# rsokolovskii/fl_scaling_sc_ldpc

Measured on AMD Instinct MI355X. Metric: MC codeword trials/sec, (4,8) SC-LDPC L=50 N=1000 eps=0.48 full BP, higher is better.
Workload: dtype u32

## Files before the change

### fl_scaling_sc_ldpc_amd/csrc/full_bp_small.hip

```cpp
#include "common.h"
#include "kernel_util.h"
#include <algorithm>
#include <cstdlib>
#include <type_traits>

namespace {

using namespace scldpc_dev;

enum { SC_NE = 0, SC_REM, SC_N0, SC_N1, SC_OVF, SC_Q, SC_N = 8 };
enum { LV_VALID = 2, LV_EXTRA0 = 3, LV_PUSH = 6, LV_DROP = 9, LV_REM = 12, LV_OVF = 15, LV_N = 18 };

struct SmArgs {
    int L, V, C, n, nk, cn_lim, nw, ncw;
    uint32_t magic_v, magic_c;
    int ntrials;
    int kswitch;
    int max_it;
    int rows_cap;
    int32_t *rows;
    int off_U, off_q0, off_q1, off_pos, off_scal, off_fb, total, qcap;
    const uint16_t *vn_adj16;
    const uint16_t *cn_adj16;
    const uint32_t *chan;
    int32_t *counters;
    uint32_t *erased_out;
    int ncaps;
    int caps[SCLDPC_MAX_CAPS];
};

template <int BLOCK, bool LEVEL, bool PERSIST, bool SOCK, bool TRAJ = false, bool CAPS = false, bool WIDE = false>
__global__ __launch_bounds__(BLOCK, WIDE ? 4 : PERSIST ? 8 : 7) __attribute__((amdgpu_num_sgpr(96))) void full_bp_small_kernel(const SmArgs a)
{
    static_assert(!WIDE || (BLOCK == 1024 && LEVEL && SOCK && !PERSIST && !CAPS), "the wide form: LEVEL [+ TRAJ], socket table");
    using QT = std::conditional_t<WIDE, uint32_t, uint16_t>;
    constexpr int kWaves = BLOCK / 64;
    extern __shared__ uint32_t lds[];
    uint32_t *cnt = lds;
    uint32_t *U = lds + a.off_U;
    QT *q[2] = {reinterpret_cast<QT *>(lds + a.off_q0), reinterpret_cast<QT *>(lds + a.off_q1)};
    int *pos_cnt = reinterpret_cast<int *>(lds + a.off_pos);
    int *pos_ss = pos_cnt + a.L;
    int *scal = reinterpret_cast<int *>(lds + a.off_scal);

    const int tid = threadIdx.x, lane = tid & 63, wave = tid >> 6;
    auto decode_trial = [&](const int trial) {
    STAMP_DECL
    const int n = a.n, nk = a.nk, cn_lim = a.cn_lim, nw = a.nw, V = a.V, C = a.C, L = a.L, qcap = a.qcap;
    const uint2 *vrow = reinterpret_cast<const uint2 *>(a.vn_adj16) + (size_t)trial * n;
    const uint4 *crow = reinterpret_cast<const uint4 *>(a.cn_adj16) + (size_t)trial * nk;
    const uint32_t *ch = a.chan + (size_t)trial * nw;

    for (int c = tid; c < a.ncw; c += BLOCK) cnt[c] = 0;
    int ne_local = 0;
    for (int w = tid; w < nw; w += BLOCK) {
        uint32_t x = ch[w];
        if (w == nw - 1 && (n & 31)) x &= (1u << (n & 31)) - 1u;
        U[w] = x;
        ne_local += __popc(x);
    }
    if (tid < LV_N) scal[tid] = 0;
    for (int i = tid; i < 2 * L; i += BLOCK) pos_cnt[i] = 0;
    __syncthreads();
    ne_local = wave_sum(ne_local);
    if (lane == 0 && ne_local) atomicAdd(&scal[SC_NE], ne_local);

    constexpr int NB = 8;
    for (int j0 = tid; j0 < n; j0 += NB * BLOCK) {
        uint2 r[NB];
        bool er[NB];
#pragma unroll
        for (int u = 0; u < NB; u++) {
            const int j = j0 + u * BLOCK;
            er[u] = false;
            if (j < n) { r[u] = vrow[j]; er[u] = (U[j >> 5] >> (j & 31)) & 1u; }
        }
#pragma unroll
        for (int u = 0; u < NB; u++) {
            const int j = j0 + u * BLOCK;
            if (er[u]) {
                const int base = (int)__umulhi((uint32_t)j, a.magic_v) * C;
                const int c0 = base + (int)(r[u].x & 0xFFFFu), c1 = base + C + (int)(r[u].x >> 16);
                const int c2 = base + 2 * C + (int)(r[u].y & 0xFFFFu), c3 = base + 3 * C + (int)(r[u].y >> 16);
                atomicAdd(&cnt[c0 >> 3], 1u << ((c0 & 7) * 4));
                atomicAdd(&cnt[c1 >> 3], 1u << ((c1 & 7) * 4));
                atomicAdd(&cnt[c2 >> 3], 1u << ((c2 & 7) * 4));
                atomicAdd(&cnt[c3 >> 3], 1u << ((c3 & 7) * 4));
            }
        }
    }
    __syncthreads();
    STAMP(0);
    const int nch = scal[SC_NE];

    int removed = 0, drops = 0;
    auto step = [&](int c, uint32_t (&out)[4]) {
        out[0] = out[1] = out[2] = out[3] = 0;
        const uint4 s4 = crow[c];
        uint32_t jk[8] = {s4.x & 0xFFFFu, s4.x >> 16, s4.y & 0xFFFFu, s4.y >> 16,
                          s4.z & 0xFFFFu, s4.z >> 16, s4.w & 0xFFFFu, s4.w >> 16};
        bool none[8];
#pragma unroll
        for (int k = 0; k < 8; k++) none[k] = jk[k] == 0xFFFFu;
        if constexpr (SOCK) {
            const int vbase = (int)__umulhi((uint32_t)c, a.magic_c) * V;
#pragma unroll
            for (int k = 0; k < 8; k++) jk[k] = (uint32_t)(vbase - (int)(jk[k] & 3u) * V) + (jk[k] >> 2);
        }
        uint32_t wd[8];
#pragma unroll
        for (int k = 0; k < 8; k++) wd[k] = U[none[k] ? 0u : jk[k] >> 5];
        int j = -1;
#pragma unroll
        for (int k = 0; k < 8; k++)
            if (!none[k] && ((wd[k] >> (jk[k] & 31u)) & 1u)) j = (int)jk[k];
        if (j < 0) return;
        const uint2 r = vrow[j];
        const uint32_t bit = 1u << (j & 31);
        if (!(atomicAnd(&U[j >> 5], ~bit) & bit)) return;
        removed++;
        const int base = (int)__umulhi((uint32_t)j, a.magic_v) * C;
        const int cc[4] = {base + (int)(r.x & 0xFFFFu), base + C + (int)(r.x >> 16),
                           base + 2 * C + (int)(r.y & 0xFFFFu), base + 3 * C + (int)(r.y >> 16)};
        uint32_t o[4];
#pragma unroll
        for (int i = 0; i < 4; i++) o[i] = atomicSub(&cnt[cc[i] >> 3], 1u << ((cc[i] & 7) * 4));
#pragma unroll
        for (int i = 0; i < 4; i++) {
            const uint32_t old = (o[i] >> ((cc[i] & 7) * 4)) & 15u;
            if (old == 2u && cc[i] < cn_lim) out[i] = (uint32_t)cc[i] + 1u;
            if constexpr (LEVEL) drops += (old == 1u && cc[i] < cn_lim);
        }
    };
    auto ones_of = [&](int w) {
        const uint32_t y = cnt[w] ^ 0x11111111u;
        uint32_t z = ~(((y & 0x77777777u) + 0x77777777u) | y) & 0x88888888u;
        if (w * 8 + 8 > cn_lim) {
            const int keep = cn_lim - w * 8;
            z = keep <= 0 ? 0u : (z & ((1u << (4 * keep)) - 1u));
        }
        return z;
    };
    auto append = [&](const uint32_t (&out)[4], int *push, QT *qn, bool &overflow) {
        const int mine = (out[0] != 0u) + (out[1] != 0u) + (out[2] != 0u) + (out[3] != 0u);
        const int incl = (int)wave_inclusive_scan((uint32_t)mine);
        const int tot = __builtin_amdgcn_readlane(incl, 63);
        if (tot) {
            int base = 0;
            if (lane == 0) base = atomicAdd(push, tot);
            int idx = __builtin_amdgcn_readfirstlane(base) + incl - mine;
#pragma unroll
            for (int i = 0; i < 4; i++)
                if (out[i]) { if (idx < qcap) qn[idx] = (QT)(out[i] - 1u); else overflow = true; idx++; }
        }
    };

    int rounds = 0, ne = 0, status = 0, be = 0, ee = 0, bee = 0;
    auto residual = [&]() {
    if (ne > 0) {
        for (int w = tid; w < nw; w += BLOCK) {
            uint32_t x = U[w];
            int p0 = (int)__umulhi((uint32_t)(w * 32), a.magic_v);
            int room = (p0 + 1) * V - w * 32;
            while (x) {
                const uint32_t lo = room >= 32 ? x : (x & ((1u << room) - 1u));
                if (lo) atomicAdd(&pos_cnt[p0], __popc(lo));
                x = room >= 32 ? 0u : (x >> room);
                p0++;
                room = V;
            }
        }
        __syncthreads();
        int q0 = 0;
        for (;;) {
            while (q0 < L && pos_cnt[q0] == 0) q0++;
            if (q0 >= L) break;
            for (int t = tid; t < V; t += BLOCK) {
                const int j = q0 * V + t;
                if (!((U[j >> 5] >> (j & 31)) & 1u)) continue;
                const uint2 r = vrow[j];
                const int base = q0 * C;
                const int cc[4] = {base + (int)(r.x & 0xFFFFu), base + C + (int)(r.x >> 16),
                                   base + 2 * C + (int)(r.y & 0xFFFFu), base + 3 * C + (int)(r.y >> 16)};
                bool pair = true;
#pragma unroll
                for (int i = 0; i < 4; i++) pair = pair && ((cnt[cc[i] >> 3] >> ((cc[i] & 7) * 4)) & 15u) == 2u;
                if (!pair) continue;
                int partner = -1;
                for (int i = 0; i < 4 && pair; i++) {
                    const uint4 s4 = crow[cc[i]];
                    const uint32_t jk[8] = {s4.x & 0xFFFFu, s4.x >> 16, s4.y & 0xFFFFu, s4.y >> 16,
                                            s4.z & 0xFFFFu, s4.z >> 16, s4.w & 0xFFFFu, s4.w >> 16};
                    int other = -1;
                    for (int k = 0; k < 8; k++) {
                        if (jk[k] == 0xFFFFu) continue;
                        const int j2 = SOCK ? (q0 + i - (int)(jk[k] & 3u)) * V + (int)(jk[k] >> 2) : (int)jk[k];
                        if (j2 != j && ((U[j2 >> 5] >> (j2 & 31)) & 1u)) other = j2;
                    }
                    if (other < 0 || (i > 0 && other != partner)) pair = false;
                    partner = other;
                }
                if (pair && (int)__umulhi((uint32_t)partner, a.magic_v) == q0) atomicAdd(&pos_ss[q0], 1);
            }
            __syncthreads();
            const int e = pos_cnt[q0] - pos_ss[q0];
            if (e > 0) { ee = e; bee = 1; break; }
            q0++;
        }
        for (int pos = 0; pos < L; pos++) be += pos_cnt[pos] > 0;
    }
    };
    auto put = [&](int32_t *o, int ne, int be, int ee, int bee, int rounds, int status) {
        o[SCLDPC_C_NUM_ERASURES] = ne;
        o[SCLDPC_C_NUM_BLOCKS_ERR] = be;
        o[SCLDPC_C_NUM_ERASURES_EXP] = ee;
        o[SCLDPC_C_NUM_BLOCKS_ERR_EXP] = bee;
        o[SCLDPC_C_NUM_ERASURES_P1] = 0;
        o[SCLDPC_C_ITERATIONS] = rounds;
        o[SCLDPC_C_STATUS] = status;
        o[SCLDPC_C_CHANNEL_ERASURES] = nch;
    };
    auto cap_counters = [&](int k) { return a.counters + ((size_t)k * a.ntrials + trial) * SCLDPC_NCOUNTERS; };

    int ci = 0;
    if constexpr (LEVEL) {
        uint8_t *fb = reinterpret_cast<uint8_t *>(lds + a.off_fb);
        int prec = n, iter = 0, ncur = 0, nfront = 0, first_word = 0;
        if constexpr (TRAJ) {
            int extra = 0;
            const int head = 3 * C, tail0 = L * C;
            for (int i = tid; i < 2 * head; i += BLOCK) {
                const int c = i < head ? i : tail0 + (i - head);
                if (c >= cn_lim || c >= nk) continue;
                const uint4 s4 = crow[c];
                const int deg = ((s4.x & 0xFFFFu) != 0xFFFFu) + ((s4.x >> 16) != 0xFFFFu) + ((s4.y & 0xFFFFu) != 0xFFFFu) +
                                ((s4.y >> 16) != 0xFFFFu) + ((s4.z & 0xFFFFu) != 0xFFFFu) + ((s4.z >> 16) != 0xFFFFu) +
                                ((s4.w & 0xFFFFu) != 0xFFFFu) + ((s4.w >> 16) != 0xFFFFu);
                extra += deg == 1 && ((cnt[c >> 3] >> ((c & 7) * 4)) & 15u) == 0u;
            }
            extra = wave_sum(extra);
            if (lane == 0 && extra) atomicAdd(&scal[LV_EXTRA0], extra);
        }
        bool scan = true;
        ne = nch;
        for (;;) {
            const int g = iter % 3, gn = (iter + 1) % 3;
            QT *qc = q[iter & 1], *qn = q[(iter + 1) & 1];
            if (tid == 0) { scal[LV_PUSH + gn] = 0; scal[LV_DROP + gn] = 0; scal[LV_REM + gn] = 0; scal[LV_OVF + gn] = 0; }
            int *push = &scal[LV_PUSH + g];
            bool overflow = false;
            removed = 0; drops = 0;
            auto run_queue = [&](int nq) {
                for (int k0 = wave * 64; k0 < nq; k0 += BLOCK) {
                    uint32_t out[4] = {0, 0, 0, 0};
                    if (k0 + lane < nq) step((int)qc[k0 + lane], out);
                    append(out, push, qn, overflow);
                }
            };
            if (scan) {
                int valid = 0;
                for (int w = tid; w < a.ncw; w += BLOCK) {
                    uint32_t y = ones_of(w) >> 3;
                    y = (y | (y >> 3)) & 0x03030303u;
                    y = (y | (y >> 6)) & 0x000F000Fu;
                    y = (y | (y >> 12)) & 0xFFu;
                    fb[w] = (uint8_t)y;
                    valid += __popc(y);
                }
                if (iter == 0) {
                    valid = wave_sum(valid);
                    if (lane == 0 && valid) atomicAdd(&scal[LV_VALID], valid);
                }
                if (tid == 0) scal[SC_Q] = 0;
                __syncthreads();
                if (iter == 0) nfront = scal[LV_VALID];
                for (;;) {
                    for (int w0 = wave * 64; w0 < a.ncw; w0 += BLOCK) {
                        const int w = w0 + lane;
                        uint32_t y = w < a.ncw ? (uint32_t)fb[w] : 0u;
                        const int mine = __popc(y);
                        const int incl = (int)wave_inclusive_scan((uint32_t)mine);
                        const int tot = __builtin_amdgcn_readlane(incl, 63);
                        if (tot == 0) continue;
                        int base = 0;
                        if (lane == 0) base = atomicAdd(&scal[SC_Q], tot);
                        int idx = __builtin_amdgcn_readfirstlane(base) + incl - mine;
                        uint32_t left = 0;
                        while (y) {
                            const int k = __ffs((int)y) - 1;
                            y &= y - 1;
                            if (idx < qcap) qc[idx] = (QT)(w * 8 + k); else left |= 1u << k;
                            idx++;
                        }
                        if (mine) fb[w] = (uint8_t)left;
                    }
                    __syncthreads();
                    const int found = scal[SC_Q];
                    __syncthreads();
                    if (tid == 0) scal[SC_Q] = 0;
                    run_queue(min(found, qcap));
                    if (found <= qcap) break;
                    __syncthreads();
                }
            } else {
                run_queue(ncur);
            }
            STAMP(4);
            {
                const uint32_t both = (uint32_t)wave_sum((int)((uint32_t)removed | ((uint32_t)drops << 15)));
                removed = (int)(both & 0x7FFFu); drops = (int)(both >> 15);
            }
            if (lane == 0) {
                if (removed) atomicAdd(&scal[LV_REM + g], removed);
                if (drops) atomicAdd(&scal[LV_DROP + g], drops);
            }
            if (overflow) scal[LV_OVF + g] = 1;
            STAMP(5);
            __syncthreads();
            STAMP(6);
            const int deg1 = nfront + ((TRAJ && iter == 0) ? scal[LV_EXTRA0] : 0);
            ne -= scal[LV_REM + g];
            const int recovered = prec - ne;
            if constexpr (TRAJ) {
                if (wave == 0 && a.rows && rounds < a.rows_cap) {
                    int fw = first_word, first = n;
                    while (fw < nw) {
                        const uint32_t w = (fw + lane < nw) ? U[fw + lane] : 0u;
                        const unsigned long long m = __ballot(w != 0u);
                        if (m) {
                            const int l0 = __ffsll((long long)m) - 1;
                            const uint32_t w0 = (uint32_t)__shfl((int)w, l0, 64);
                            fw += l0;
                            first = fw * 32 + (__ffs((int)w0) - 1);
                            break;
                        }
                        fw += 64;
                    }
                    first_word = fw;
                    if (lane == 0) {
                        int32_t *r = a.rows + ((size_t)trial * a.rows_cap + rounds) * 3;
                        r[0] = deg1; r[1] = recovered; r[2] = (int)__umulhi((uint32_t)first, a.magic_v);
                    }
                }
                __syncthreads();
            }
            rounds++;
            if (deg1 < recovered && iter > 0) { status = -1; break; }
            if (ne == 0 || ne == prec) break;
            prec = ne;
            nfront = scal[LV_PUSH + g] - (scal[LV_DROP + g] - nfront);
            scan = scal[LV_OVF + g] != 0;
            ncur = scan ? 0 : scal[LV_PUSH + g];
            iter++;
            if (!CAPS && a.max_it > 0 && iter >= a.max_it) break;
            if constexpr (CAPS) {
                if (iter >= a.caps[ci]) {
                    be = ee = bee = 0;
                    residual();
                    if (tid == 0) put(cap_counters(ci), ne, be, ee, bee, rounds, 0);
                    __syncthreads();
                    for (int i = tid; i < 2 * L; i += BLOCK) pos_cnt[i] = 0;
                    if (++ci == a.ncaps) break;
                }
            }
            STAMP(7);
        }
        __syncthreads();
        STAMP(1);
    } else {
        const int kSwitch = a.kswitch;
        const int wcap = (qcap / kWaves) & ~1, half_cap = wcap / 2;
        int ncur = 0;
        bool scan = true;
        for (;;) {
            QT *qc = q[rounds & 1], *qn = q[(rounds + 1) & 1];
            if (scan) {
                for (int w0 = wave * 64; w0 < a.ncw; w0 += BLOCK) {
                    const int w = w0 + lane;
                    uint32_t z = w < a.ncw ? ones_of(w) : 0u;
                    const int mine = __popc(z);
                    const int incl = (int)wave_inclusive_scan((uint32_t)mine);
                    const int tot = __builtin_amdgcn_readlane(incl, 63);
                    if (tot == 0) continue;
                    int base = 0;
                    if (lane == 0) base = atomicAdd(&scal[SC_Q], tot);
                    base = __builtin_amdgcn_readfirstlane(base);
                    int idx = base + incl - mine;
                    while (z) {
                        const int k = (__ffs((int)z) - 1) >> 2;
                        z &= z - 1;
                        if (idx < qcap) qc[idx] = (QT)(w * 8 + k);
                        idx++;
                    }
                }
                __syncthreads();
                ncur = scal[SC_Q];
                if (ncur > qcap) { ncur = qcap; if (tid == 0) scal[SC_OVF] = 1; }
                __syncthreads();
            }
            if (tid == 0) { scal[SC_Q] = 0; scal[SC_N0 + ((rounds + 1) & 1)] = 0; }
            int *push = &scal[SC_N0 + (rounds & 1)];
            bool overflow = false;
            if (ncur > kSwitch || half_cap < 64) {
                for (int k0 = wave * 64; k0 < ncur; k0 += BLOCK) {
                    uint32_t out[4] = {0, 0, 0, 0};
                    if (k0 + lane < ncur) step((int)qc[k0 + lane], out);
                    append(out, push, qn, overflow);
                }
            } else {
                QT *mine = qn + wave * wcap;
                int cntw = (ncur - wave + kWaves - 1) / kWaves, cur = 0;
                if (cntw < 0) cntw = 0;
                if (lane < cntw) mine[lane] = qc[wave + lane * kWaves];
                while (cntw > 0) {
                    QT *src = mine + cur * half_cap, *dst = mine + (cur ^ 1) * half_cap;
                    int ncnt = 0;
                    for (int b0 = 0; b0 < cntw; b0 += 64) {
                        uint32_t out[4] = {0, 0, 0, 0};
                        if (b0 + lane < cntw) step((int)src[b0 + lane], out);
                        {
                            const int mine_n = (out[0] != 0u) + (out[1] != 0u) + (out[2] != 0u) + (out[3] != 0u);
                            const int incl = (int)wave_inclusive_scan((uint32_t)mine_n);
                            int idx = ncnt + incl - mine_n;
    #pragma unroll
                            for (int i = 0; i < 4; i++)
                                if (out[i]) { if (idx < half_cap) dst[idx] = (QT)(out[i] - 1u); else overflow = true; idx++; }
                            ncnt += __builtin_amdgcn_readlane(incl, 63);
                        }
                    }
                    cntw = min(ncnt, half_cap);
                    cur ^= 1;
                }
            }
            if (overflow) scal[SC_OVF] = 1;
            __syncthreads();
            rounds++;
            const int pushed = *push;
            scan = scal[SC_OVF] != 0;
            __syncthreads();
            if (tid == 0) scal[SC_OVF] = 0;
            ncur = scan ? 0 : min(pushed, qcap);
            if (!scan && ncur == 0) break;
        }
        STAMP(1);
        removed = wave_sum(removed);
        if (lane == 0 && removed) atomicAdd(&scal[SC_REM], removed);
        __syncthreads();
        ne = nch - scal[SC_REM];
    }

    if (!CAPS || ci < a.ncaps) {
        be = ee = bee = 0;
        residual();
    }
    STAMP(2);
    STAMP_FLUSH();
    if (a.erased_out)
        for (int w = tid; w < nw; w += BLOCK) a.erased_out[(size_t)trial * nw + w] = U[w];
    if (tid == 0) {
        if constexpr (CAPS) {
            for (int k = ci; k < a.ncaps; k++) put(cap_counters(k), ne, be, ee, bee, rounds, status);
        } else {
            put(a.counters + (size_t)trial * SCLDPC_NCOUNTERS, ne, be, ee, bee, rounds, status);
        }
    }
    };
    if constexpr (PERSIST) {
        for (int trial = blockIdx.x; trial < a.ntrials; trial += gridDim.x) {
            decode_trial(trial);
            __syncthreads();
        }
    } else {
        decode_trial((int)blockIdx.x);
    }
}

int make_args(const scldpc_code_params *p, int32_t is_term, SmArgs *a, int per_cu, bool level = false, bool wide = false)
{
    const int n = scldpc::n_of(p), nk = scldpc::nk_of(p);
    a->L = p->L; a->V = p->vns_pos; a->C = p->cns_pos; a->n = n; a->nk = nk;
    a->cn_lim = is_term ? nk : p->L * p->cns_pos;
    a->nw = (n + 31) / 32; a->ncw = (nk + 7) / 8;
    int off = 0;
    auto take = [&](int words) { int o = off; off += (words + 3) & ~3; return o; };
    take(a->ncw);
    a->off_U = take(a->nw);
    a->off_pos = take(2 * p->L);
    a->off_scal = take(LV_N);
    a->off_fb = level ? take((a->ncw + 3) / 4) : 0;
    const int budget = scldpc::kMaxLdsBytes / per_cu / 4 - 128;
    int qwords = ((budget - off) / 2) & ~3;
    if (qwords > 2048 && !wide) qwords = 2048;
    if (qwords < 128) return -1;
    a->qcap = wide ? qwords : 2 * qwords;
    a->off_q0 = take(qwords);
    a->off_q1 = take(qwords);
    a->total = off;
    return 0;
}

constexpr int kBlockSmall = 256;
constexpr int kPerCu = 7;
constexpr int kSwitchWidth = 128;
constexpr int kBlockWide = 1024;
constexpr int kWideMinQueue = 1024;
static_assert(kSwitchWidth <= 64 * (kBlockSmall / 64), "a wave takes at most one frontier entry per lane into its private queue");

}

namespace {
bool small_shape(const scldpc_code_params *p)
{
    if (scldpc::check_params(p)) return false;
    SmArgs a{};
    uint32_t m;
    return p->dv == 4 && p->dc == 8 && p->cns_pos <= 65536 && scldpc::nk_of(p) <= 65536 &&
           make_args(p, 1, &a, 1) == 0 && scldpc::magic_of(p->vns_pos, scldpc::n_of(p) + 32, &m) &&
           scldpc::magic_of(p->cns_pos, scldpc::nk_of(p), &m);
}
}

namespace {
const char *wide_limit(const scldpc_code_params *p)
{
    if (scldpc::check_params(p)) return "invalid code parameters";
    if (p->dv != 4 || p->dc != 8) return "takes dv = 4, dc = 8 only";
    if ((int64_t)p->vns_pos * p->dv > 65535) return "sockets: vns_pos * dv must fit 16 bits (at most 65535)";
    if (p->cns_pos > 65536) return "sockets: at most 65536 CNs per position (16-bit position-local CN ids)";
    const int64_t n64 = (int64_t)p->L * p->vns_pos, nk64 = (int64_t)(p->L + p->dv - 1) * p->cns_pos;
    if (n64 / 8 + nk64 / 2 > scldpc::kMaxLdsBytes) return "LDS: the CN counts and VN bits of a trial exceed 160 KiB";
    SmArgs a{};
    uint32_t m;
    if (!scldpc::magic_of(p->vns_pos, scldpc::n_of(p) + 32, &m) || !scldpc::magic_of(p->cns_pos, scldpc::nk_of(p), &m))
        return "no exact multiply-high division for this vns_pos / cns_pos";
    if (make_args(p, 1, &a, 1, true, true) != 0) return "LDS: the CN counts and VN bits of a trial leave no room for the queues";
    if (a.qcap < kWideMinQueue) return "queue: the LDS left by the state holds fewer than 1024 entries per queue";
    if (a.nk / 16 + 64 * (a.nk / a.qcap + 1) > 32767) return "queue: a wave's releases per iteration could exceed 15 bits";
    return nullptr;
}
}

extern "C" int scldpc_full_bp_wide_supported(const scldpc_code_params *p)
{
    return wide_limit(p) == nullptr;
}

extern "C" int scldpc_full_bp_cn16_supported(const scldpc_code_params *p)
{
    return small_shape(p) && scldpc::n_of(p) < 65535;
}

extern "C" int scldpc_full_bp_sock16_supported(const scldpc_code_params *p)
{
    return small_shape(p) && (int64_t)p->vns_pos * p->dv <= 65535;
}

namespace {

int launch_small(const char *who, bool level, bool sock, const scldpc_code_params *p, int32_t ntrials, const uint16_t *d_vn_adj16,
                 const uint16_t *d_cn_adj16, const uint32_t *d_chan_bits, int32_t max_it, int32_t is_term,
                 int32_t *d_counters, uint32_t *d_erased_bits, void *stream, int32_t *d_rows = nullptr, int32_t rows_cap = 0)
{
    if (d_rows && (rows_cap <= 0 || !level))
        return scldpc::set_error(SCLDPC_ERR_BAD_ARG, "%s: d_rows given but rows_cap <= 0", who);
    if (int rc = scldpc::check_params(p)) return rc;
    if (!(sock ? scldpc_full_bp_sock16_supported(p) : scldpc_full_bp_cn16_supported(p)))
        return scldpc::set_error(SCLDPC_ERR_TOO_LARGE, "%s: takes dv = 4, dc = 8, at most 65536 CNs per trial%s", who,
                                 sock ? " and 16-bit sockets" : " and fewer than 65535 VNs (use the _sock16 form beyond)");
    if (ntrials < 0 || (ntrials > 0 && (!d_counters || !d_vn_adj16 || !d_cn_adj16 || !d_chan_bits)))
        return scldpc::set_error(SCLDPC_ERR_BAD_ARG, "%s: null buffer or negative ntrials", who);
    if (ntrials == 0) return SCLDPC_OK;
    SmArgs a{};
    int per_cu = kPerCu;
    while (per_cu > 1 && make_args(p, is_term, &a, per_cu, level) != 0) per_cu--;
    if (make_args(p, is_term, &a, per_cu, level) != 0)
        return scldpc::set_error(SCLDPC_ERR_TOO_LARGE, "%s: the CN counts and VN bits do not fit the LDS", who);
    scldpc::magic_of(p->vns_pos, a.n + 32, &a.magic_v);
    scldpc::magic_of(p->cns_pos, a.nk, &a.magic_c);
    a.vn_adj16 = d_vn_adj16; a.cn_adj16 = d_cn_adj16; a.chan = d_chan_bits;
    a.counters = d_counters; a.erased_out = d_erased_bits;
    a.kswitch = kSwitchWidth;
    if (const char *v = getenv("SCLDPC_DEBUG_DECODER_KSWITCH")) a.kswitch = std::min(atoi(v), 64 * (kBlockSmall / 64));
    a.ntrials = ntrials;
    a.rows = d_rows; a.rows_cap = d_rows ? rows_cap : 0;
    a.max_it = max_it;
    const int grid = scldpc::debug_grid("DECODER", ntrials);
    void (*kern)(const SmArgs) = sock ? (level ? full_bp_small_kernel<kBlockSmall, true, false, true> : full_bp_small_kernel<kBlockSmall, false, false, true>)
        : grid < ntrials ? (level ? full_bp_small_kernel<kBlockSmall, true, true, false> : full_bp_small_kernel<kBlockSmall, false, true, false>)
                         : (level ? full_bp_small_kernel<kBlockSmall, true, false, false> : full_bp_small_kernel<kBlockSmall, false, false, false>);
    if (sock && grid < ntrials) return scldpc::set_error(SCLDPC_ERR_BAD_ARG, "%s: no persistent form with the socket table", who);
    if (d_rows) kern = sock ? full_bp_small_kernel<kBlockSmall, true, false, true, true> : full_bp_small_kernel<kBlockSmall, true, false, false, true>;
    size_t lds_bytes = 4u * (size_t)a.total;
    lds_bytes = std::min(lds_bytes + scldpc::debug_lds_pad("DECODER"), (size_t)scldpc::kMaxLdsBytes);
    if (int rc_ = scldpc::allow_max_lds(reinterpret_cast<const void *>(kern))) return rc_;
    hipLaunchKernelGGL(kern, dim3(grid), dim3(kBlockSmall), lds_bytes, static_cast<hipStream_t>(stream), a);
    SCLDPC_HIP_CHECK(hipGetLastError());
    return SCLDPC_OK;
}

int launch_caps(const char *who, bool sock, const scldpc_code_params *p, int32_t ntrials, const uint16_t *d_vn_adj16,
                const uint16_t *d_cn_adj16, const uint32_t *d_chan_bits, int32_t ncaps, const int32_t *caps, int32_t is_term,
                int32_t *d_counters, void *stream)
{
    if (ncaps < 1 || ncaps > SCLDPC_MAX_CAPS || !caps)
        return scldpc::set_error(SCLDPC_ERR_BAD_ARG, "%s: takes 1 .. %d caps (ncaps = %d%s)", who, SCLDPC_MAX_CAPS, ncaps,
                                 caps ? "" : ", caps NULL");
    for (int k = 0; k < ncaps; k++)
        if (caps[k] < 1 || (k > 0 && caps[k] <= caps[k - 1]))
            return scldpc::set_error(SCLDPC_ERR_BAD_ARG, "%s: caps must be strictly increasing and >= 1 (caps[%d] = %d)", who, k,
                                     caps[k]);
    if (ntrials < 0 || (ntrials > 0 && (!d_counters || !d_vn_adj16 || !d_cn_adj16 || !d_chan_bits)))
        return scldpc::set_error(SCLDPC_ERR_BAD_ARG, "%s: null buffer or negative ntrials", who);
    if (int rc = scldpc::check_params(p)) return rc;
    if (!(sock ? scldpc_full_bp_sock16_supported(p) : scldpc_full_bp_cn16_supported(p)))
        return scldpc::set_error(SCLDPC_ERR_TOO_LARGE, "%s: takes dv = 4, dc = 8, at most 65536 CNs per trial%s", who,
                                 sock ? " and 16-bit sockets" : " and fewer than 65535 VNs (use the _sock16 form beyond)");
    if (ntrials == 0) return SCLDPC_OK;
    SmArgs a{};
    int per_cu = kPerCu;
    while (per_cu > 1 && make_args(p, is_term, &a, per_cu, true) != 0) per_cu--;
    if (make_args(p, is_term, &a, per_cu, true) != 0)
        return scldpc::set_error(SCLDPC_ERR_TOO_LARGE, "%s: the CN counts and VN bits do not fit the LDS", who);
    scldpc::magic_of(p->vns_pos, a.n + 32, &a.magic_v);
    scldpc::magic_of(p->cns_pos, a.nk, &a.magic_c);
    a.vn_adj16 = d_vn_adj16; a.cn_adj16 = d_cn_adj16; a.chan = d_chan_bits;
    a.counters = d_counters;
    a.kswitch = kSwitchWidth;
    a.ntrials = ntrials;
    a.ncaps = ncaps;
    for (int k = 0; k < ncaps; k++) a.caps[k] = caps[k];
    void (*kern)(const SmArgs) = sock ? full_bp_small_kernel<kBlockSmall, true, false, true, false, true>
                                      : full_bp_small_kernel<kBlockSmall, true, false, false, false, true>;
    const size_t lds_bytes = 4u * (size_t)a.total;
    if (int rc_ = scldpc::allow_max_lds(reinterpret_cast<const void *>(kern))) return rc_;
    hipLaunchKernelGGL(kern, dim3(ntrials), dim3(kBlockSmall), lds_bytes, static_cast<hipStream_t>(stream), a);
    SCLDPC_HIP_CHECK(hipGetLastError());
    return SCLDPC_OK;
}

int launch_wide(const char *who, const scldpc_code_params *p, int32_t ntrials, const uint16_t *d_vn_adj16,
                const uint16_t *d_cn_sock16, const uint32_t *d_chan_bits, int32_t max_it, int32_t is_term,
                int32_t *d_counters, uint32_t *d_erased_bits, void *stream, int32_t *d_rows, int32_t rows_cap)
{
    if (d_rows && rows_cap <= 0) return scldpc::set_error(SCLDPC_ERR_BAD_ARG, "%s: d_rows given but rows_cap <= 0", who);
    if (int rc = scldpc::check_params(p)) return rc;
    if (const char *why = wide_limit(p)) return scldpc::set_error(SCLDPC_ERR_TOO_LARGE, "%s: %s", who, why);
    if (ntrials < 0 || (ntrials > 0 && (!d_counters || !d_vn_adj16 || !d_cn_sock16 || !d_chan_bits)))
        return scldpc::set_error(SCLDPC_ERR_BAD_ARG, "%s: null buffer or negative ntrials", who);
    if (ntrials == 0) return SCLDPC_OK;
    SmArgs a{};
    if (make_args(p, is_term, &a, 1, true, true) != 0 || 4u * (size_t)a.total > (size_t)scldpc::kMaxLdsBytes)
        return scldpc::set_error(SCLDPC_ERR_TOO_LARGE, "%s: LDS: the CN counts and VN bits do not fit", who);
    scldpc::magic_of(p->vns_pos, a.n + 32, &a.magic_v);
    scldpc::magic_of(p->cns_pos, a.nk, &a.magic_c);
    a.vn_adj16 = d_vn_adj16; a.cn_adj16 = d_cn_sock16; a.chan = d_chan_bits;
    a.counters = d_counters; a.erased_out = d_erased_bits;
    a.kswitch = kSwitchWidth;
    a.ntrials = ntrials;
    a.rows = d_rows; a.rows_cap = d_rows ? rows_cap : 0;
    a.max_it = max_it;
    void (*kern)(const SmArgs) = d_rows ? full_bp_small_kernel<kBlockWide, true, false, true, true, false, true>
                                        : full_bp_small_kernel<kBlockWide, true, false, true, false, false, true>;
    const size_t lds_bytes = 4u * (size_t)a.total;
    if (int rc_ = scldpc::allow_max_lds(reinterpret_cast<const void *>(kern))) return rc_;
    hipLaunchKernelGGL(kern, dim3(ntrials), dim3(kBlockWide), lds_bytes, static_cast<hipStream_t>(stream), a);
    SCLDPC_HIP_CHECK(hipGetLastError());
    return SCLDPC_OK;
}

}

extern "C" int scldpc_full_bp_device_wide(const scldpc_code_params *p, int32_t ntrials, const uint16_t *d_vn_adj16,
                                          const uint16_t *d_cn_sock16, const uint32_t *d_chan_bits, int32_t max_it,
                                          int32_t is_term, int32_t *d_counters, uint32_t *d_erased_bits, void *stream)
{
    return launch_wide("scldpc_full_bp_device_wide", p, ntrials, d_vn_adj16, d_cn_sock16, d_chan_bits, max_it, is_term,
                       d_counters, d_erased_bits, stream, nullptr, 0);
}

extern "C" int scldpc_full_bp_traj_device_wide(const scldpc_code_params *p, int32_t ntrials, const uint16_t *d_vn_adj16,
                                               const uint16_t *d_cn_sock16, const uint32_t *d_chan_bits, int32_t max_it,
                                               int32_t is_term, int32_t *d_counters, int32_t *d_rows, int32_t rows_cap,
                                               uint32_t *d_erased_bits, void *stream)
{
    if (!d_rows) return scldpc::set_error(SCLDPC_ERR_BAD_ARG, "scldpc_full_bp_traj_device_wide: null d_rows");
    return launch_wide("scldpc_full_bp_traj_device_wide", p, ntrials, d_vn_adj16, d_cn_sock16, d_chan_bits, max_it, is_term,
                       d_counters, d_erased_bits, stream, d_rows, rows_cap);
}

extern "C" int scldpc_full_bp_fixpoint_device_cn16(const scldpc_code_params *p, int32_t ntrials,
                                                   const uint16_t *d_vn_adj16, const uint16_t *d_cn_adj16,
                                                   const uint32_t *d_chan_bits, int32_t is_term, int32_t *d_counters,
                                                   uint32_t *d_erased_bits, void *stream)
{
    return launch_small("scldpc_full_bp_fixpoint_device_cn16", false, false, p, ntrials, d_vn_adj16, d_cn_adj16, d_chan_bits, 0,
                        is_term, d_counters, d_erased_bits, stream);
}

extern "C" int scldpc_full_bp_device_cn16(const scldpc_code_params *p, int32_t ntrials, const uint16_t *d_vn_adj16,
                                          const uint16_t *d_cn_adj16, const uint32_t *d_chan_bits, int32_t max_it,
                                          int32_t is_term, int32_t *d_counters, uint32_t *d_erased_bits, void *stream)
{
    return launch_small("scldpc_full_bp_device_cn16", true, false, p, ntrials, d_vn_adj16, d_cn_adj16, d_chan_bits, max_it,
                        is_term, d_counters, d_erased_bits, stream);
}

extern "C" int scldpc_full_bp_fixpoint_device_sock16(const scldpc_code_params *p, int32_t ntrials,
                                                     const uint16_t *d_vn_adj16, const uint16_t *d_cn_sock16,
                                                     const uint32_t *d_chan_bits, int32_t is_term, int32_t *d_counters,
                                                     uint32_t *d_erased_bits, void *stream)
{
    return launch_small("scldpc_full_bp_fixpoint_device_sock16", false, true, p, ntrials, d_vn_adj16, d_cn_sock16, d_chan_bits,
                        0, is_term, d_counters, d_erased_bits, stream);
}

extern "C" int scldpc_full_bp_device_sock16(const scldpc_code_params *p, int32_t ntrials, const uint16_t *d_vn_adj16,
                                            const uint16_t *d_cn_sock16, const uint32_t *d_chan_bits, int32_t max_it,
                                            int32_t is_term, int32_t *d_counters, uint32_t *d_erased_bits, void *stream)
{
    return launch_small("scldpc_full_bp_device_sock16", true, true, p, ntrials, d_vn_adj16, d_cn_sock16, d_chan_bits, max_it,
                        is_term, d_counters, d_erased_bits, stream);
}

extern "C" int scldpc_full_bp_traj_device_cn16(const scldpc_code_params *p, int32_t ntrials, const uint16_t *d_vn_adj16,
                                               const uint16_t *d_cn_adj16, const uint32_t *d_chan_bits, int32_t max_it,
                                               int32_t is_term, int32_t *d_counters, int32_t *d_rows, int32_t rows_cap,
                                               uint32_t *d_erased_bits, void *stream)
{
    if (!d_rows) return scldpc::set_error(SCLDPC_ERR_BAD_ARG, "scldpc_full_bp_traj_device_cn16: null d_rows");
    return launch_small("scldpc_full_bp_traj_device_cn16", true, false, p, ntrials, d_vn_adj16, d_cn_adj16, d_chan_bits, max_it,
                        is_term, d_counters, d_erased_bits, stream, d_rows, rows_cap);
}

extern "C" int scldpc_full_bp_traj_device_sock16(const scldpc_code_params *p, int32_t ntrials, const uint16_t *d_vn_adj16,
                                                 const uint16_t *d_cn_sock16, const uint32_t *d_chan_bits, int32_t max_it,
                                                 int32_t is_term, int32_t *d_counters, int32_t *d_rows, int32_t rows_cap,
                                                 uint32_t *d_erased_bits, void *stream)
{
    if (!d_rows) return scldpc::set_error(SCLDPC_ERR_BAD_ARG, "scldpc_full_bp_traj_device_sock16: null d_rows");
    return launch_small("scldpc_full_bp_traj_device_sock16", true, true, p, ntrials, d_vn_adj16, d_cn_sock16, d_chan_bits, max_it,
                        is_term, d_counters, d_erased_bits, stream, d_rows, rows_cap);
}

extern "C" int scldpc_full_bp_caps_device_cn16(const scldpc_code_params *p, int32_t ntrials, const uint16_t *d_vn_adj16,
                                               const uint16_t *d_cn_adj16, const uint32_t *d_chan_bits, int32_t ncaps,
                                               const int32_t *caps, int32_t is_term, int32_t *d_counters, void *stream)
{
    return launch_caps("scldpc_full_bp_caps_device_cn16", false, p, ntrials, d_vn_adj16, d_cn_adj16, d_chan_bits, ncaps, caps,
                       is_term, d_counters, stream);
}

extern "C" int scldpc_full_bp_caps_device_sock16(const scldpc_code_params *p, int32_t ntrials, const uint16_t *d_vn_adj16,
                                                 const uint16_t *d_cn_sock16, const uint32_t *d_chan_bits, int32_t ncaps,
                                                 const int32_t *caps, int32_t is_term, int32_t *d_counters, void *stream)
{
    return launch_caps("scldpc_full_bp_caps_device_sock16", true, p, ntrials, d_vn_adj16, d_cn_sock16, d_chan_bits, ncaps, caps,
                       is_term, d_counters, stream);
}
```

Measured before the change: 1.218 million.

## Build CN erasure counts per check row and seed peeling queue with degree-one VNs

In the non-level, non-socket fixpoint form, the initial CN erasure counters are now built by each thread reading its check-node row, gathering the erased bits of its neighbours, and packing eight 4-bit counts per word with DPP lane merges. This replaces the per-erased-VN atomicAdd scatter. The same pass finds degree-one checks and writes their single erased VN id straight into the first queue, so the first peeling round skips the counter scan and starts from a VN list. The cost is reading every CN row even when few VNs are erased, plus a new template variant. An environment variable can switch back to the old build.

Result: no change. 1.221 million, median of 6 (+0.3%).

```diff
diff --git a/fl_scaling_sc_ldpc_amd/csrc/full_bp_small.hip b/fl_scaling_sc_ldpc_amd/csrc/full_bp_small.hip
--- a/fl_scaling_sc_ldpc_amd/csrc/full_bp_small.hip
+++ b/fl_scaling_sc_ldpc_amd/csrc/full_bp_small.hip
@@ -2,13 +2,14 @@
 #include "kernel_util.h"
 #include <algorithm>
 #include <cstdlib>
+#include <cstring>
 #include <type_traits>
 
 namespace {
 
 using namespace scldpc_dev;
 
-enum { SC_NE = 0, SC_REM, SC_N0, SC_N1, SC_OVF, SC_Q, SC_N = 8 };
+enum { SC_NE = 0, SC_REM, SC_N0, SC_N1, SC_OVF, SC_Q, SC_B, SC_N = 8 };
 enum { LV_VALID = 2, LV_EXTRA0 = 3, LV_PUSH = 6, LV_DROP = 9, LV_REM = 12, LV_OVF = 15, LV_N = 18 };
 
 struct SmArgs {
@@ -29,10 +30,11 @@
     int caps[SCLDPC_MAX_CAPS];
 };
 
-template <int BLOCK, bool LEVEL, bool PERSIST, bool SOCK, bool TRAJ = false, bool CAPS = false, bool WIDE = false>
+template <int BLOCK, bool LEVEL, bool PERSIST, bool SOCK, bool TRAJ = false, bool CAPS = false, bool WIDE = false, bool CNB = false>
 __global__ __launch_bounds__(BLOCK, WIDE ? 4 : PERSIST ? 8 : 7) __attribute__((amdgpu_num_sgpr(96))) void full_bp_small_kernel(const SmArgs a)
 {
     static_assert(!WIDE || (BLOCK == 1024 && LEVEL && SOCK && !PERSIST && !CAPS), "the wide form: LEVEL [+ TRAJ], socket table");
+    static_assert(!CNB || (!LEVEL && !SOCK && !WIDE && BLOCK % 64 == 0), "the CN-row build: fixpoint form, 16-bit VN ids as queue entries");
     using QT = std::conditional_t<WIDE, uint32_t, uint16_t>;
     constexpr int kWaves = BLOCK / 64;
     extern __shared__ uint32_t lds[];
@@ -51,7 +53,8 @@
     const uint4 *crow = reinterpret_cast<const uint4 *>(a.cn_adj16) + (size_t)trial * nk;
     const uint32_t *ch = a.chan + (size_t)trial * nw;
 
-    for (int c = tid; c < a.ncw; c += BLOCK) cnt[c] = 0;
+    if constexpr (!CNB)
+        for (int c = tid; c < a.ncw; c += BLOCK) cnt[c] = 0;
     int ne_local = 0;
     for (int w = tid; w < nw; w += BLOCK) {
         uint32_t x = ch[w];
@@ -65,6 +68,65 @@
     ne_local = wave_sum(ne_local);
     if (lane == 0 && ne_local) atomicAdd(&scal[SC_NE], ne_local);
 
+    if constexpr (CNB) {
+    constexpr int NB = 4;
+    QT *q0 = q[0];
+    const int nk8 = a.ncw * 8;
+    for (int b = 0; b < nk8; b += NB * BLOCK) {
+        uint4 r[NB];
+#pragma unroll
+        for (int u = 0; u < NB; u++) {
+            const int c = b + u * BLOCK + tid;
+            r[u] = make_uint4(~0u, ~0u, ~0u, ~0u);
+            if (c < nk) r[u] = crow[c];
+        }
+        auto tally = [&](auto full, const uint4 &s4, uint32_t &count, uint32_t &j1) {
+            const uint32_t jk[8] = {s4.x & 0xFFFFu, s4.x >> 16, s4.y & 0xFFFFu, s4.y >> 16,
+                                    s4.z & 0xFFFFu, s4.z >> 16, s4.w & 0xFFFFu, s4.w >> 16};
+            uint32_t wd[8];
+#pragma unroll
+            for (int k = 0; k < 8; k++) wd[k] = U[(decltype(full)::value || jk[k] != 0xFFFFu) ? jk[k] >> 5 : 0u];
+            count = 0; j1 = 0;
+#pragma unroll
+            for (int k = 0; k < 8; k++) {
+                const bool set = (decltype(full)::value || jk[k] != 0xFFFFu) && ((wd[k] >> (jk[k] & 31u)) & 1u);
+                count += set;
+                j1 = set ? jk[k] : j1;
+            }
+        };
+        bool one[NB];
+        uint32_t j1[NB];
+#pragma unroll
+        for (int u = 0; u < NB; u++) {
+            const int c = b + u * BLOCK + tid;
+            const int cw = b + u * BLOCK + __builtin_amdgcn_readfirstlane(wave) * 64;
+            uint32_t count;
+            if (cw >= 3 * C && cw + 64 <= L * C) tally(std::true_type{}, r[u], count, j1[u]);
+            else tally(std::false_type{}, r[u], count, j1[u]);
+            uint32_t v = count << ((lane & 7) * 4);
+            v |= (uint32_t)__builtin_amdgcn_update_dpp(0, (int)v, 0xB1, 0xF, 0xF, false);
+            v |= (uint32_t)__builtin_amdgcn_update_dpp(0, (int)v, 0x4E, 0xF, 0xF, false);
+            v |= (uint32_t)__builtin_amdgcn_update_dpp(0, (int)v, 0x141, 0xF, 0xF, false);
+            if ((lane & 7) == 0 && c < nk8) cnt[c >> 3] = v;
+            one[u] = count == 1u && c < cn_lim;
+        }
+        unsigned long long m[NB];
+        int tot = 0;
+#pragma unroll
+        for (int u = 0; u < NB; u++) { m[u] = __ballot(one[u]); tot += __popcll(m[u]); }
+        if (tot) {
+            int idx = 0;
+            if (lane == 0) idx = atomicAdd(&scal[SC_B], tot);
+            idx = __builtin_amdgcn_readfirstlane(idx);
+#pragma unroll
+            for (int u = 0; u < NB; u++) {
+                const int at = idx + (int)__builtin_amdgcn_mbcnt_hi((uint32_t)(m[u] >> 32), __builtin_amdgcn_mbcnt_lo((uint32_t)m[u], 0u));
+                if (one[u] && at < qcap) q0[at] = (QT)j1[u];
+                idx += __popcll(m[u]);
+            }
+        }
+    }
+    } else {
     constexpr int NB = 8;
     for (int j0 = tid; j0 < n; j0 += NB * BLOCK) {
         uint2 r[NB];
@@ -89,33 +151,13 @@
             }
         }
     }
+    }
     __syncthreads();
     STAMP(0);
     const int nch = scal[SC_NE];
 
     int removed = 0, drops = 0;
-    auto step = [&](int c, uint32_t (&out)[4]) {
-        out[0] = out[1] = out[2] = out[3] = 0;
-        const uint4 s4 = crow[c];
-        uint32_t jk[8] = {s4.x & 0xFFFFu, s4.x >> 16, s4.y & 0xFFFFu, s4.y >> 16,
-                          s4.z & 0xFFFFu, s4.z >> 16, s4.w & 0xFFFFu, s4.w >> 16};
-        bool none[8];
-#pragma unroll
-        for (int k = 0; k < 8; k++) none[k] = jk[k] == 0xFFFFu;
-        if constexpr (SOCK) {
-            const int vbase = (int)__umulhi((uint32_t)c, a.magic_c) * V;
-#pragma unroll
-            for (int k = 0; k < 8; k++) jk[k] = (uint32_t)(vbase - (int)(jk[k] & 3u) * V) + (jk[k] >> 2);
-        }
-        uint32_t wd[8];
-#pragma unroll
-        for (int k = 0; k < 8; k++) wd[k] = U[none[k] ? 0u : jk[k] >> 5];
-        int j = -1;
-#pragma unroll
-        for (int k = 0; k < 8; k++)
-            if (!none[k] && ((wd[k] >> (jk[k] & 31u)) & 1u)) j = (int)jk[k];
-        if (j < 0) return;
-        const uint2 r = vrow[j];
+    auto release = [&](int j, const uint2 r, uint32_t (&out)[4]) {
         const uint32_t bit = 1u << (j & 31);
         if (!(atomicAnd(&U[j >> 5], ~bit) & bit)) return;
         removed++;
@@ -131,6 +173,33 @@
             if (old == 2u && cc[i] < cn_lim) out[i] = (uint32_t)cc[i] + 1u;
             if constexpr (LEVEL) drops += (old == 1u && cc[i] < cn_lim);
         }
+    };
+    auto step = [&](int c, uint32_t (&out)[4]) {
+        out[0] = out[1] = out[2] = out[3] = 0;
+        const uint4 s4 = crow[c];
+        uint32_t jk[8] = {s4.x & 0xFFFFu, s4.x >> 16, s4.y & 0xFFFFu, s4.y >> 16,
+                          s4.z & 0xFFFFu, s4.z >> 16, s4.w & 0xFFFFu, s4.w >> 16};
+        bool none[8];
+#pragma unroll
+        for (int k = 0; k < 8; k++) none[k] = jk[k] == 0xFFFFu;
+        if constexpr (SOCK) {
+            const int vbase = (int)__umulhi((uint32_t)c, a.magic_c) * V;
+#pragma unroll
+            for (int k = 0; k < 8; k++) jk[k] = (uint32_t)(vbase - (int)(jk[k] & 3u) * V) + (jk[k] >> 2);
+        }
+        uint32_t wd[8];
+#pragma unroll
+        for (int k = 0; k < 8; k++) wd[k] = U[none[k] ? 0u : jk[k] >> 5];
+        int j = -1;
+#pragma unroll
+        for (int k = 0; k < 8; k++)
+            if (!none[k] && ((wd[k] >> (jk[k] & 31u)) & 1u)) j = (int)jk[k];
+        if (j < 0) return;
+        release(j, vrow[j], out);
+    };
+    auto step_vn = [&](int j, uint32_t (&out)[4]) {
+        out[0] = out[1] = out[2] = out[3] = 0;
+        release(j, vrow[j], out);
     };
     auto ones_of = [&](int w) {
         const uint32_t y = cnt[w] ^ 0x11111111u;
@@ -371,7 +440,12 @@
         const int kSwitch = a.kswitch;
         const int wcap = (qcap / kWaves) & ~1, half_cap = wcap / 2;
         int ncur = 0;
-        bool scan = true;
+        bool scan = true, vn_list = false;
+        if constexpr (CNB) {
+            ncur = scal[SC_B];
+            if (ncur > qcap) { ncur = qcap; if (tid == 0) scal[SC_OVF] = 1; }
+            scan = false; vn_list = true;
+        }
         for (;;) {
             QT *qc = q[rounds & 1], *qn = q[(rounds + 1) & 1];
             if (scan) {
@@ -401,12 +475,15 @@
             if (tid == 0) { scal[SC_Q] = 0; scal[SC_N0 + ((rounds + 1) & 1)] = 0; }
             int *push = &scal[SC_N0 + (rounds & 1)];
             bool overflow = false;
-            if (ncur > kSwitch || half_cap < 64) {
+            if (vn_list || ncur > kSwitch || half_cap < 64) {
                 for (int k0 = wave * 64; k0 < ncur; k0 += BLOCK) {
                     uint32_t out[4] = {0, 0, 0, 0};
-                    if (k0 + lane < ncur) step((int)qc[k0 + lane], out);
+                    if (k0 + lane < ncur) {
+                        if (CNB && vn_list) step_vn((int)qc[k0 + lane], out); else step((int)qc[k0 + lane], out);
+                    }
                     append(out, push, qn, overflow);
                 }
+                vn_list = false;
             } else {
                 QT *mine = qn + wave * wcap;
                 int cntw = (ncur - wave + kWaves - 1) / kWaves, cur = 0;
@@ -556,6 +633,11 @@
 }
 
 namespace {
+
+bool cn_row_build_off(const char *v)
+{
+    return v && (!strcmp(v, "vn") || !strcmp(v, "0"));
+}
 
 int launch_small(const char *who, bool level, bool sock, const scldpc_code_params *p, int32_t ntrials, const uint16_t *d_vn_adj16,
                  const uint16_t *d_cn_adj16, const uint32_t *d_chan_bits, int32_t max_it, int32_t is_term,
@@ -589,6 +671,9 @@
         : grid < ntrials ? (level ? full_bp_small_kernel<kBlockSmall, true, true, false> : full_bp_small_kernel<kBlockSmall, false, true, false>)
                          : (level ? full_bp_small_kernel<kBlockSmall, true, false, false> : full_bp_small_kernel<kBlockSmall, false, false, false>);
     if (sock && grid < ntrials) return scldpc::set_error(SCLDPC_ERR_BAD_ARG, "%s: no persistent form with the socket table", who);
+    if (!level && !sock && !cn_row_build_off(getenv("SCLDPC_DEBUG_DECODER_BUILD")))
+        kern = grid < ntrials ? full_bp_small_kernel<kBlockSmall, false, true, false, false, false, false, true>
+                              : full_bp_small_kernel<kBlockSmall, false, false, false, false, false, false, true>;
     if (d_rows) kern = sock ? full_bp_small_kernel<kBlockSmall, true, false, true, true> : full_bp_small_kernel<kBlockSmall, true, false, false, true>;
     size_t lds_bytes = 4u * (size_t)a.total;
     lds_bytes = std::min(lds_bytes + scldpc::debug_lds_pad("DECODER"), (size_t)scldpc::kMaxLdsBytes);
```
